# cocowy1/PPMStereo

Hardware: AMD Instinct MI355X
Metric: disparity-px/s (higher is better)
Workload: dtype bf16; 1 GPU; BASELINE config 2: T=5 clip at 320x512, iters=10, hot path only (3-scale cascade from encoder outputs: corr pyramid build + lookup, QAM pick, pick-and-play memory attention, ConvGRU3D update, heads, convex upsample, test_mode=True as PPMStereo.forward_batch_test calls it: predictions[-1] is the output, so the mask head, the convex upsampling and the full-resolution resize run only where their resu; T=5, H=320, W=512, iters=10, parallelism=replicas x1

## Files before the change

### include/ppms.h

```cpp
#ifndef PPMS_H
#define PPMS_H
#include <stdint.h>

#ifdef __cplusplus
extern "C" {
#endif

#define PPMS_OK 0
#define PPMS_EINVAL (-1)
#define PPMS_ELAUNCH (-2)
#define PPMS_ENODEV (-3)

#define PPMS_ABI_VERSION 4

int ppms_version(void);
const char* ppms_last_error(void);
int ppms_device_info(char* name, int name_cap, int* cu_count, int* clock_mhz);

int ppms_corr_build(const float* fmap1, const float* fmap2, float* const pyr[5], int B, int C, int H, int W, void* stream);

int ppms_corr_lookup(const float* const pyr[4], const float* flow, int flow_nhwc, float* out_nchw, void* out_hi, void* out_lo,
                     int out_ld, void* flow_sp_hi, void* flow_sp_lo, int flow_sp_ld, int B, int H, int W, void* stream);

typedef struct ppms_sp {
// ... 42 lines not shown
    int32_t lo_zero_from;
    ppms_epilogue epi[2];
} ppms_conv;

int ppms_conv_gemm2(const ppms_conv* desc, const ppms_conv* dev_desc, int wm_hint, void* stream);
int ppms_conv_gemm2_slices(const ppms_conv* desc);
int64_t ppms_conv_gemm2_slice_workspace_bytes(const ppms_conv* desc, int nslice);
int ppms_conv_gemm2_sliced(const ppms_conv* desc, const ppms_conv* dev_desc, int nslice, void* workspace, void* stream);
int ppms_conv_gemm2_ysweep_slices(const ppms_conv* desc);
int ppms_conv_gemm2_ysweep(const ppms_conv* desc, const ppms_conv* dev_desc, int nslice, void* workspace, void* stream);
int ppms_conv_gemm5_applicable(const ppms_conv* desc);
int ppms_conv_gemm5(const ppms_conv* desc, const ppms_conv* dev_desc, int nbt, void* stream);
int ppms_conv_gemm5_slices(const ppms_conv* desc);
int ppms_conv_gemm5_sliced(const ppms_conv* desc, const ppms_conv* dev_desc, int nbt, int nslice, void* workspace, void* stream);
int ppms_conv_gemm6_applicable(const ppms_conv* desc);
int ppms_conv_gemm6(const ppms_conv* desc, const ppms_conv* dev_desc, void* stream);
int ppms_gemm1_applicable(const ppms_conv* desc);
int ppms_gemm1(const ppms_conv* desc, const ppms_conv* dev_desc, int cb_hint, void* stream);
int ppms_conv_stream_applicable(const ppms_conv* desc);
int ppms_conv_stream(const ppms_conv* desc, const ppms_conv* dev_desc, int hint, void* stream);
int ppms_struct_sizes(int* sp, int* epilogue, int* conv);

int ppms_dwconv_gelu(ppms_sp x, ppms_sp y, const float* w, const float* b, int k, int BT, int H, int W, void* stream);
int ppms_flow_patch7(const float* flow_nhwc, ppms_sp patch, int BT, int H, int W, void* stream);
int ppms_unc_tail(ppms_sp x, const float* w, float bias, float* unc, float* partial, int BT, int HW, void* stream);

int ppms_nchw_to_sp(const float* src, ppms_sp dst, int BT, int C, int HW, void* stream);
int ppms_sp_to_nchw(ppms_sp src, float* dst, int BT, int C, int HW, void* stream);
int ppms_nchw_to_nhwc(const float* src, float* dst, int dst_ld, int BT, int C, int HW, void* stream);
int ppms_nhwc_to_nchw(const float* src, int src_ld, float* dst, int BT, int C, int HW, void* stream);
int ppms_f32_to_sp(const float* src, int src_ld, ppms_sp dst, int64_t pixels, void* stream);
int ppms_sp_to_f32(ppms_sp src, float* dst, int dst_ld, int64_t pixels, void* stream);

int ppms_tap_gather_sum(const float* y, int y_ld, const float* bias, float* out, int out_ld, float* accum, int accum_ld, int cout, int kt, int kh,
                        int kw, int T, int H, int W, int t_halo, void* stream);
int ppms_flow_add(float* flow_nhwc, const float* dflow, int dflow_ld, int64_t pixels, void* stream);
int ppms_convex_upsample(const float* flow_nhwc, const float* mask, int mask_ld, float* out, int BT, int H, int W, void* stream);
int ppms_convex_upsample_3d(const float* flow_nhwc, const float* mask, int mask_ld, float* out, int T, int H, int W, int t_halo, void* stream);
int ppms_bilinear(const float* src, float* dst, int N, int C, int H, int W, int OH, int OW, int align_corners, float mul, void* stream);

int ppms_sp_resize_blend(ppms_sp src, ppms_sp dst, int N, int H, int W, int OH, int OW, float a, float b, void* stream);

int ppms_avgpool(const float* src, float* dst, int planes, int H, int W, int k, void* stream);
int ppms_axpby(const float* x, const float* y, float* out, float a, float b, int64_t period, int64_t n, void* stream);
int ppms_ctx_mix(const float* fmap, const float* ctx, float* net, float* inp, int N, int HW, void* stream);

int ppms_img_s2d(const float* img_nchw, ppms_sp dst, int N, int C, int H, int W, int k, void* stream);
int ppms_sp_s2d(ppms_sp src, ppms_sp dst, int N, int H, int W, void* stream);
int ppms_video_ingest_u8(const uint8_t* left, const uint8_t* right, int64_t frame_stride, int N, int H0, int W0, int pad_left, int pad_top, int H, int W,
                         const float* lut, ppms_sp dst_fnet, ppms_sp dst_cnet, void* stream);
int64_t ppms_instnorm_workspace_bytes(int N, int HW, int C);
int ppms_instnorm_stats(const float* x, int ld, int N, int HW, int C, float eps, float* stats, void* workspace, void* stream);
int ppms_instnorm_apply(const float* x, int ld, const float* stats, ppms_sp res, int relu, ppms_sp out, int N, int HW, int C, void* stream);

int ppms_dwconv(ppms_sp x, float* y, int ldy, const float* w, const float* b, int k, int N, int H, int W, void* stream);
int ppms_layernorm_any(const float* x, int ld, const float* w, const float* b, float eps, ppms_sp out, int64_t pixels, int C, void* stream);
int64_t ppms_grn_workspace_bytes(int N, int HW, int C);
int ppms_grn(const float* x, int ld, const float* gamma, const float* beta, ppms_sp out, int N, int HW, int C, void* workspace, void* stream);
int ppms_sp_upsample2(ppms_sp src, ppms_sp dst, int N, int H, int W, void* stream);

int ppms_qk_similarity(const float* q, const float* k, int ld, float* pooled, float* sim, int T, int H, int W, void* stream);
int ppms_qk_pool(const float* q, const float* k, int ld, float* pooled, int T, int H, int W, void* stream);
int ppms_qk_cos(const float* pooled, float* sim, int T, int cells, void* stream);
int ppms_qam_select(const float* sim, float* strive, const float* conf_partial, int nblk, int HW, int32_t* sel, float* shat,
                    float* score, int T, void* stream);
int ppms_attn_prep_q(const float* q, int ld, const float* pe, void* qb, int T, int n, void* stream);
int ppms_attn_prep_k(const float* key, int ld, const float* pe, const int32_t* sel, const float* shat, void* kb, int T, int ksel,
                     int n, void* stream);
enum { PPMS_ATTN_P_BF16 = 0, PPMS_ATTN_P_FP16 = 1 };
int ppms_mem_attn(const void* qb, const void* kb, const void* vt, const int32_t* sel, int ksel, float scale, const float* beta,
                  ppms_sp mf, ppms_sp mfg, void* out_bf16, int T, int n, void* split_ws, int frames_per_workgroup, int p_format, void* stream);
int64_t ppms_mem_attn_workspace_bytes(int T, int ksel, int n);
int ppms_mem_attn_splits(int T, int ksel, int n, int frames_per_workgroup);
int ppms_attn_redo_accumulate(const void* split_ws, int T, int ksel, int n, int frames_per_workgroup, int64_t* counters, void* stream);

int ppms_pwchain(const void* dev_params, int64_t pixels, void* stream);
int ppms_pwchain_param_bytes(void);

int ppms_time_attn(ppms_sp x, const float* ln_w, const float* ln_b, ppms_sp out, int T, int n, int heads, void* stream);
int ppms_layernorm(const float* x, int ld, const float* w, const float* b, ppms_sp resid, ppms_sp out, int64_t pixels, int C, void* stream);
int64_t ppms_linear_attention_workspace_floats(int T, int n, int heads, int dh);
int ppms_linear_attention(const float* Q, int ldq, const float* K, int ldk, const float* V, int ldv, float* kv_ws, ppms_sp out, int T, int n,
                          int heads, int dh, void* stream);

#ifdef __cplusplus
}
#endif
#endif
```

### ppmstereo_amd/_lib.py

```python
from __future__ import annotations

import ctypes as C
import os
from typing import Optional

import torch

from . import build as _build

c_void_p, c_int, c_float, c_int64 = C.c_void_p, C.c_int, C.c_float, C.c_int64

EPI_STORE, EPI_RESID, EPI_RH, EPI_GRU, EPI_ADDF32 = range(5)
ATTN_P_BF16, ATTN_P_FP16 = 0, 1
ACT_NONE, ACT_RELU, ACT_GELU, ACT_SIGMOID, ACT_TANH, ACT_ELU1 = range(6)


def vt_image(v: torch.Tensor, p_format: int) -> torch.Tensor:
    b = v.to(torch.bfloat16)
    if p_format == ATTN_P_BF16:
        return b.contiguous()
    return b.float().clamp(-65504.0, 65504.0).to(torch.float16).contiguous().view(torch.bfloat16)


def vt_values(vt: torch.Tensor, p_format: int) -> torch.Tensor:
# ... 32 lines not shown
    "ppms_last_error": (C.c_char_p, []),
    "ppms_device_info": (c_int, [C.c_char_p, c_int, C.POINTER(c_int), C.POINTER(c_int)]),
    "ppms_corr_build": (c_int, [c_void_p, c_void_p, C.POINTER(c_void_p), c_int, c_int, c_int, c_int, c_void_p]),
    "ppms_corr_lookup": (c_int, [C.POINTER(c_void_p), c_void_p, c_int, c_void_p, c_void_p, c_void_p, c_int, c_void_p, c_void_p,
                                 c_int, c_int, c_int, c_int, c_void_p]),
    "ppms_conv_gemm2": (c_int, [C.POINTER(Conv), c_void_p, c_int, c_void_p]),
    "ppms_conv_gemm2_slices": (c_int, [C.POINTER(Conv)]),
    "ppms_conv_gemm2_slice_workspace_bytes": (C.c_int64, [C.POINTER(Conv), c_int]),
    "ppms_conv_gemm2_sliced": (c_int, [C.POINTER(Conv), c_void_p, c_int, c_void_p, c_void_p]),
    "ppms_conv_gemm2_ysweep_slices": (c_int, [C.POINTER(Conv)]),
    "ppms_conv_gemm2_ysweep": (c_int, [C.POINTER(Conv), c_void_p, c_int, c_void_p, c_void_p]),
    "ppms_gemm1_applicable": (c_int, [C.POINTER(Conv)]),
    "ppms_gemm1": (c_int, [C.POINTER(Conv), c_void_p, c_int, c_void_p]),
    "ppms_conv_stream_applicable": (c_int, [C.POINTER(Conv)]),
    "ppms_conv_stream": (c_int, [C.POINTER(Conv), c_void_p, c_int, c_void_p]),
    "ppms_conv_gemm5_applicable": (c_int, [C.POINTER(Conv)]),
    "ppms_conv_gemm5": (c_int, [C.POINTER(Conv), c_void_p, c_int, c_void_p]),
    "ppms_conv_gemm6_applicable": (c_int, [C.POINTER(Conv)]),
    "ppms_conv_gemm6": (c_int, [C.POINTER(Conv), c_void_p, c_void_p]),
    "ppms_conv_gemm5_slices": (c_int, [C.POINTER(Conv)]),
    "ppms_conv_gemm5_sliced": (c_int, [C.POINTER(Conv), c_void_p, c_int, c_int, c_void_p, c_void_p]),
    "ppms_struct_sizes": (c_int, [C.POINTER(c_int), C.POINTER(c_int), C.POINTER(c_int)]),
    "ppms_dwconv_gelu": (c_int, [SP, SP, c_void_p, c_void_p, c_int, c_int, c_int, c_int, c_void_p]),
    "ppms_flow_patch7": (c_int, [c_void_p, SP, c_int, c_int, c_int, c_void_p]),
    "ppms_unc_tail": (c_int, [SP, c_void_p, c_float, c_void_p, c_void_p, c_int, c_int, c_void_p]),
    "ppms_nchw_to_sp": (c_int, [c_void_p, SP, c_int, c_int, c_int, c_void_p]),
    "ppms_sp_to_nchw": (c_int, [SP, c_void_p, c_int, c_int, c_int, c_void_p]),
    "ppms_nchw_to_nhwc": (c_int, [c_void_p, c_void_p, c_int, c_int, c_int, c_int, c_void_p]),
    "ppms_nhwc_to_nchw": (c_int, [c_void_p, c_int, c_void_p, c_int, c_int, c_int, c_void_p]),
    "ppms_f32_to_sp": (c_int, [c_void_p, c_int, SP, c_int64, c_void_p]),
    "ppms_sp_to_f32": (c_int, [SP, c_void_p, c_int, c_int64, c_void_p]),
    "ppms_tap_gather_sum": (c_int, [c_void_p, c_int, c_void_p, c_void_p, c_int, c_void_p, c_int, c_int, c_int, c_int, c_int, c_int, c_int, c_int, c_int, c_void_p]),
    "ppms_flow_add": (c_int, [c_void_p, c_void_p, c_int, c_int64, c_void_p]),
    "ppms_convex_upsample": (c_int, [c_void_p, c_void_p, c_int, c_void_p, c_int, c_int, c_int, c_void_p]),
    "ppms_convex_upsample_3d": (c_int, [c_void_p, c_void_p, c_int, c_void_p, c_int, c_int, c_int, c_int, c_void_p]),
    "ppms_bilinear": (c_int, [c_void_p, c_void_p, c_int, c_int, c_int, c_int, c_int, c_int, c_int, c_float, c_void_p]),
    "ppms_sp_resize_blend": (c_int, [SP, SP, c_int, c_int, c_int, c_int, c_int, c_float, c_float, c_void_p]),
    "ppms_avgpool": (c_int, [c_void_p, c_void_p, c_int, c_int, c_int, c_int, c_void_p]),
    "ppms_axpby": (c_int, [c_void_p, c_void_p, c_void_p, c_float, c_float, c_int64, c_int64, c_void_p]),
    "ppms_ctx_mix": (c_int, [c_void_p, c_void_p, c_void_p, c_void_p, c_int, c_int, c_void_p]),
    "ppms_img_s2d": (c_int, [c_void_p, SP, c_int, c_int, c_int, c_int, c_int, c_void_p]),
    "ppms_video_ingest_u8": (c_int, [c_void_p, c_void_p, c_int64, c_int, c_int, c_int, c_int, c_int, c_int, c_int, c_void_p, SP, SP, c_void_p]),
    "ppms_dwconv": (c_int, [SP, c_void_p, c_int, c_void_p, c_void_p, c_int, c_int, c_int, c_int, c_void_p]),
    "ppms_layernorm_any": (c_int, [c_void_p, c_int, c_void_p, c_void_p, c_float, SP, c_int64, c_int, c_void_p]),
    "ppms_grn_workspace_bytes": (c_int64, [c_int, c_int, c_int]),
    "ppms_grn": (c_int, [c_void_p, c_int, c_void_p, c_void_p, SP, c_int, c_int, c_int, c_void_p, c_void_p]),
    "ppms_sp_upsample2": (c_int, [SP, SP, c_int, c_int, c_int, c_void_p]),
    "ppms_sp_s2d": (c_int, [SP, SP, c_int, c_int, c_int, c_void_p]),
    "ppms_instnorm_workspace_bytes": (c_int64, [c_int, c_int, c_int]),
    "ppms_instnorm_stats": (c_int, [c_void_p, c_int, c_int, c_int, c_int, C.c_float, c_void_p, c_void_p, c_void_p]),
    "ppms_instnorm_apply": (c_int, [c_void_p, c_int, c_void_p, SP, c_int, SP, c_int, c_int, c_int, c_void_p]),
    "ppms_qk_similarity": (c_int, [c_void_p, c_void_p, c_int, c_void_p, c_void_p, c_int, c_int, c_int, c_void_p]),
    "ppms_qk_pool": (c_int, [c_void_p, c_void_p, c_int, c_void_p, c_int, c_int, c_int, c_void_p]),
    "ppms_qk_cos": (c_int, [c_void_p, c_void_p, c_int, c_int, c_void_p]),
    "ppms_qam_select": (c_int, [c_void_p, c_void_p, c_void_p, c_int, c_int, c_void_p, c_void_p, c_void_p, c_int, c_void_p]),
    "ppms_attn_prep_q": (c_int, [c_void_p, c_int, c_void_p, c_void_p, c_int, c_int, c_void_p]),
    "ppms_attn_prep_k": (c_int, [c_void_p, c_int, c_void_p, c_void_p, c_void_p, c_void_p, c_int, c_int, c_int, c_void_p]),
    "ppms_pwchain": (c_int, [c_void_p, c_int64, c_void_p]),
    "ppms_pwchain_param_bytes": (c_int, []),
    "ppms_time_attn": (c_int, [SP, c_void_p, c_void_p, SP, c_int, c_int, c_int, c_void_p]),
    "ppms_layernorm": (c_int, [c_void_p, c_int, c_void_p, c_void_p, SP, SP, c_int64, c_int, c_void_p]),
    "ppms_linear_attention_workspace_floats": (c_int64, [c_int, c_int, c_int, c_int]),
    "ppms_linear_attention": (c_int, [c_void_p, c_int, c_void_p, c_int, c_void_p, c_int, c_void_p, SP, c_int, c_int, c_int, c_int, c_void_p]),
    "ppms_mem_attn": (c_int, [c_void_p, c_void_p, c_void_p, c_void_p, c_int, c_float, c_void_p, SP, SP, c_void_p, c_int, c_int, c_void_p, c_int, c_int, c_void_p]),
    "ppms_mem_attn_workspace_bytes": (c_int64, [c_int, c_int, c_int]),
    "ppms_mem_attn_splits": (c_int, [c_int, c_int, c_int, c_int]),
    "ppms_attn_redo_accumulate": (c_int, [c_void_p, c_int, c_int, c_int, c_int, c_void_p, c_void_p]),
}
EXPORTS = tuple(_SIGS)

_lib: Optional[C.CDLL] = None


def lib_path() -> str:
    return _build.LIB


def load() -> C.CDLL:
    global _lib
    if _lib is not None:
# ... 71 lines not shown
```

### ppmstereo_amd/csrc/small_ops.hip

```cpp
#include "common.h"

static thread_local char g_err[512] = "";
void ppms_set_error(const char* fmt, ...) {
    va_list ap;
    va_start(ap, fmt);
    vsnprintf(g_err, sizeof(g_err), fmt, ap);
    va_end(ap);
}
int ppms_check_launch(const char* what) {
    hipError_t e = hipGetLastError();
    if (e != hipSuccess) {
        ppms_set_error("%s: HIP launch failed: %s", what, hipGetErrorString(e));
        return PPMS_ELAUNCH;
    }
    return PPMS_OK;
}
extern "C" const char* ppms_last_error(void) { return g_err; }
extern "C" int ppms_version(void) { return PPMS_ABI_VERSION; }
extern "C" int ppms_struct_sizes(int* sp, int* epilogue, int* conv) {
    if (sp) *sp = (int)sizeof(ppms_sp);
    if (epilogue) *epilogue = (int)sizeof(ppms_epilogue);
    if (conv) *conv = (int)sizeof(ppms_conv);
    return PPMS_OK;
}
// ... 76 lines not shown
            const f32x4 w0 = *(const f32x4*)(wl + (ky * K + kx) * C + c0), w1 = *(const f32x4*)(wl + (ky * K + kx) * C + c0 + 4);
#pragma unroll
            for (int p = 0; p < DW_PX; ++p)
#pragma unroll
                for (int j = 0; j < 8; ++j) acc[p][j] += (j < 4 ? w0[j & 3] : w1[j & 3]) * win[p + kx][j];
        }
    }
#pragma unroll
    for (int p = 0; p < DW_PX; ++p) {
        if (px0 + p >= W) break;
        bf16x8 oh, ol;
#pragma unroll
        for (int j = 0; j < 8; ++j) {
            bf16_t hi, lo;
            split_bf16(gelu_erf(x0[p][j] + acc[p][j]), hi, lo);
            oh[j] = hi;
            ol[j] = lo;
        }
        *(bf16x8*)((bf16_t*)y.hi + (pix0 + p) * y.ld + c0) = oh;
        *(bf16x8*)((bf16_t*)y.lo + (pix0 + p) * y.ld + c0) = ol;
    }
}

extern "C" int ppms_dwconv_gelu(ppms_sp x, ppms_sp y, const float* w, const float* b, int k, int BT, int H, int W, void* stream) {
    PPMS_REQUIRE(k == 1 || k == 7, "dwconv_gelu: k=%d (only 1 and 7)", k);
    PPMS_REQUIRE(x.hi && x.lo && y.hi && y.lo && x.c == y.c && x.c > 0 && x.c <= 64 && x.c % 8 == 0 && x.ld % 8 == 0 && y.ld % 8 == 0,
                 "dwconv_gelu: views must have c <= 64 and c, ld multiples of 8");
    const int64_t rows = (int64_t)BT * H;
    const int groups = x.c / 8;
    const dim3 grid(ceil_div(rows * ((W + DW_PX - 1) / DW_PX) * groups, 256));
    if (k == 1)
        hipLaunchKernelGGL(dwconv_gelu_kernel<1>, grid, dim3(256), 0, (hipStream_t)stream, x, y, w, b, H, W, rows, groups);
    else
        hipLaunchKernelGGL(dwconv_gelu_kernel<7>, grid, dim3(256), 0, (hipStream_t)stream, x, y, w, b, H, W, rows, groups);
    return ppms_check_launch("dwconv_gelu");
}

__global__ __launch_bounds__(256) void flow_patch7_kernel(const float* __restrict__ flow, ppms_sp patch, int H, int W, int64_t P) {
    const int64_t idx = (int64_t)blockIdx.x * 256 + threadIdx.x;
    if (idx >= P * 128) return;
    const int k = (int)(idx & 127);
    const int64_t pix = idx >> 7;
    float v = 0.0f;
    if (k < 98) {
        const int tap = k >> 1, c = k & 1;
        const int ky = tap / 7, kx = tap - ky * 7;
        const int px = (int)(pix % W), py = (int)((pix / W) % H);
        const int xx = px + kx - 3, yy = py + ky - 3;
        if ((unsigned)xx < (unsigned)W && (unsigned)yy < (unsigned)H) v = flow[(pix + (int64_t)(ky - 3) * W + (kx - 3)) * 2 + c];
    }
    bf16_t hi, lo;
    split_bf16(v, hi, lo);
    ((bf16_t*)patch.hi)[pix * patch.ld + k] = hi;
    ((bf16_t*)patch.lo)[pix * patch.ld + k] = lo;
}

extern "C" int ppms_flow_patch7(const float* flow_nhwc, ppms_sp patch, int BT, int H, int W, void* stream) {
    PPMS_REQUIRE(flow_nhwc && patch.hi && patch.lo && patch.ld >= 128, "flow_patch7: bad arguments");
// ... 616 lines not shown
    const int cs = (int)(r / n);
    const int clip = cs / ksel, slot = cs - clip * ksel;
    const int frame = sel[clip * 5 + slot];
    const float s = shat[clip * 5 + slot];
    const float* kp = key + ((int64_t)frame * n + pin) * ld + g * 8;
    const f32x4 a = *(const f32x4*)kp, b = *(const f32x4*)(kp + 4);
    const f32x4 pa = *(const f32x4*)(pe + frame * 128 + g * 8), pb = *(const f32x4*)(pe + frame * 128 + g * 8 + 4);
    bf16x8 o;
#pragma unroll
    for (int j = 0; j < 4; ++j) {
        o[j] = (bf16_t)(a[j] * s + pa[j]);
        o[4 + j] = (bf16_t)(b[j] * s + pb[j]);
    }
    *(bf16x8*)(kb + r * 128 + g * 8) = o;
}
extern "C" int ppms_attn_prep_k(const float* key, int ld, const float* pe, const int32_t* sel, const float* shat, void* kb, int T, int ksel,
                                int n, void* stream) {
    PPMS_REQUIRE(key && pe && sel && shat && kb && ksel >= 1 && ksel <= 5 && ld % 4 == 0, "attn_prep_k: bad arguments");
    const int64_t total = (int64_t)T * ksel * n * 16;
    hipLaunchKernelGGL(attn_prep_k_kernel, dim3(ceil_div(total, 256)), dim3(256), 0, (hipStream_t)stream, key, ld, pe, sel, shat,
                       (bf16_t*)kb, ksel, n, total);
    return ppms_check_launch("attn_prep_k");
}
```

### ppmstereo_amd/engine.py

```python
from __future__ import annotations

import ctypes as C
import math
from typing import Dict, List, Optional

import torch

from . import _lib as L
from . import packing as _packing
from .convplan import (ALL_KERNELS, CONV2, CONV2_SWEPT, CONV6, KERNEL_TIMING, TUNING, ConvOp, PwChain, TimedCall,
                       attn_p_format, conv_desc, epilogue, pack_conv, plan_conv)

TOP_K = 5


def temporal_pe(T: int, channels: int) -> torch.Tensor:
    pos = torch.arange(T)
    pos = pos / pos[-1] * 1.0
    pos = pos.unsqueeze(1)
    div = 1.0 / (10000.0 ** (torch.arange(0, channels, 2).float() / channels))
    ang = pos * div
    pe = torch.zeros(T, channels)
    pe[:, 0::2] = torch.sin(ang)
    pe[:, 1::2] = torch.cos(ang)
# ... 9 lines not shown
    def __init__(self, sd: Dict[str, torch.Tensor], device):
        g = lambda k: sd[k].detach().to(device=device, dtype=torch.float32)
        self.w: Dict[str, dict] = {}

        def put(name, weight, bias, segs, seg_pad=None, cout_map=None, m_pad=None, kernels=ALL_KERNELS):
            self.w[name] = pack_conv(weight, bias, segs, seg_pad, cout_map, m_pad, kernels)

        e = "encoder."
        put("init0", g(e + "init_conv.0.weight"), g(e + "init_conv.0.bias"), [128])
        put("init2", g(e + "init_conv.2.weight"), g(e + "init_conv.2.bias"), [64])
        c1 = e + "convc1."
        put("ffn1_0", g(c1 + "ffn1.0.weight"), g(c1 + "ffn1.0.bias"), [36], [64], kernels=(CONV2,))
        put("ffn1_2", g(c1 + "ffn1.2.weight"), g(c1 + "ffn1.2.bias"), [54], [64], kernels=(CONV2,))
        put("pw", g(c1 + "pw.weight"), g(c1 + "pw.bias"), [36], [64], kernels=(CONV2,))
        put("ffn2_0", g(c1 + "ffn2.0.weight"), g(c1 + "ffn2.0.bias"), [36], [64], kernels=(CONV2,))
        put("ffn2_2", g(c1 + "ffn2.2.weight"), g(c1 + "ffn2.2.bias"), [54], [64], kernels=(CONV2,))
        self.dw = []
        for i, k in ((0, 1), (1, 7)):
            w = torch.zeros(64, k * k, device=device)
            b = torch.zeros(64, device=device)
            w[:36] = g(c1 + f"conv_list.{i}.weight").reshape(36, k * k)
            b[:36] = g(c1 + f"conv_list.{i}.bias")
            self.dw.append((w.contiguous(), b.contiguous(), k))
        put("convc2", g(e + "convc2.weight"), g(e + "convc2.bias"), [256])
        wf1 = g(e + "convf1.weight").permute(0, 2, 3, 1).reshape(128, 98, 1, 1)
        put("convf1", wf1, g(e + "convf1.bias"), [98], [128])
        put("convf2", g(e + "convf2.weight"), g(e + "convf2.bias"), [128])
        put("final", g(e + "final_conv.weight"), g(e + "final_conv.bias"), [320], None, list(range(126)) + list(range(128, 192)), 192)
        put("to_v", g("aggregator.to_v.weight"), None, [128])
        put("unc0", g("uncertainty.0.weight"), g("uncertainty.0.bias"), [128, 128])
        self.unc2_w = g("uncertainty.2.weight").reshape(128).contiguous()
        self.unc2_b = float(sd["uncertainty.2.bias"].detach().float().cpu().item())
        gr = "gru."
        cat = lambda a, b: torch.cat([g(a), g(b)], 0)
        put("zr1_0", cat(gr + "convz1.0.weight", gr + "convr1.0.weight"), cat(gr + "convz1.0.bias", gr + "convr1.0.bias"), [128, 384])
        put("z1_2", g(gr + "convz1.2.weight"), g(gr + "convz1.2.bias"), [128])
        put("r1_2", g(gr + "convr1.2.weight"), g(gr + "convr1.2.bias"), [128])
        self.w["zr1_2"] = {CONV6: _packing.pack_conv6_grouped([g(gr + "convz1.2.weight"), g(gr + "convr1.2.weight")], [g(gr + "convz1.2.bias"), g(gr + "convr1.2.bias")], 128)}
        put("q1", g(gr + "convq1.weight"), g(gr + "convq1.bias"), [128, 384])
        for n in ("2", "3"):
            put("zr" + n, cat(gr + f"convz{n}.weight", gr + f"convr{n}.weight"), cat(gr + f"convz{n}.bias", gr + f"convr{n}.bias"), [128, 384])
            put("q" + n, g(gr + f"convq{n}.weight"), g(gr + f"convq{n}.bias"), [128, 384])
        self.hoist = "time_attn.temporal_fc.weight" not in sd
        if self.hoist:
            for name in ("zr1_0", "q1", "zr2", "q2", "zr3", "q3"):
                if name.startswith("zr"):
# ... 66 lines not shown
            self.XG = self.X if shard is None else L.SPTensor(Tg * n, 384, device)
            self.QKF, self.VF, self.M2, self.M3 = f32(P, 768), f32(P, 384), f32(P, 384), f32(P, 384)
            self.KVWS = f32(int(L.load().ppms_linear_attention_workspace_floats(T, n, 8, 48)))
        self.Hb = [sp(128), sp(128), sp(128)]
        self.ZT, self.RT, self.RH, self.FH1, self.M1 = sp(128), sp(128), sp(128), sp(256), sp(256)
        self.Z, self.MASK, self.QK = f32(P, 128), f32(P, pk.mask_ch), f32(P, 256)
        self._FLOW_full, self._FH2Y_full = f32(P + 2 * hp, 2), f32(P + 2 * hp, 64)
        self.FLOW, self.FH2Y = self._FLOW_full[hp:hp + P], self._FH2Y_full[hp:hp + P]
        self.DFLOW = f32(P, 4)
        if pk.hoist:
            self.PRE = {k: torch.empty(P, m, dtype=torch.float32, device=device) for k, m in
                        (("zr1_0", 256), ("q1", 128), ("zr2", 256), ("q2", 128), ("zr3", 256), ("q3", 128))}
            self._pre_stream, self._ev_pre, self._pre_pending = torch.cuda.Stream(device=device), torch.cuda.Event(), False
        self.attn_p = attn_p_format()
        self.VT = torch.zeros(T, 128, n, dtype=torch.bfloat16, device=device)
        self.VTG = self.VT if shard is None else torch.zeros(Tg, 128, n, dtype=torch.bfloat16, device=device)
        self.KG = None if shard is None else f32(Tg * n, 128)
        self.QB = torch.zeros(T, n, 128, dtype=torch.bfloat16, device=device)
        self.KB = torch.zeros(T, self.ksel, n, 128, dtype=torch.bfloat16, device=device)
        self.ATT_WS = torch.empty(int(L.load().ppms_mem_attn_workspace_bytes(T, self.ksel, n)), dtype=torch.uint8, device=device)
        self.nblk = (n + 255) // 256
        self.UNC, self.PART = f32(P), f32(T, self.nblk)
        self.PARTG = self.PART if shard is None else f32(Tg, self.nblk)
        self.SIM, self.STRIVE, self.SCORE = f32(Tg, Tg), f32(Tg, Tg), f32(Tg, Tg)
        self.SEL = torch.zeros(Tg, 5, dtype=torch.int32, device=device)
        self.SHAT = f32(Tg, 5)
        self.cells = max(1, (h // 4) * (w // 4))
        self.POOL = f32(2, T, self.cells)
        self.POOLG = self.POOL if shard is None else f32(2, Tg, self.cells)
        self.PE = temporal_pe(Tg, 128).to(device)
        self.FLOW_OUT = f32(T, 2, 4 * h, 4 * w)
        self.scale = softmax_scale(128)
        self.parity = 0
        self.have_mhs = False
        self.lib = L.load()
        self._ev, self._ev_i = None, 0
        self._health, self._health_on = None, False
        self._xa_halo = None
        self._x_hid = False
        self.hbm = {"corr_lookup": TimedCall(self._lookup), "attn_prep_k": TimedCall(self._prep_k), "convex_upsample": TimedCall(self._upsample)}
        self._side = torch.cuda.Stream(device=device)
        self._ev_fork, self._ev_join = torch.cuda.Event(), torch.cuda.Event()
        self._build_descriptors()

    def _halo_sp(self, tensors, k: int, async_op: bool = False):
        if self.shard is None:
            return None
        if isinstance(tensors, L.SPTensor):
            tensors = [tensors]
        fr = self.T + 2 * self.halo
        return self.shard.halo_many([(t.data[p].view(fr, self.n, t.channels), k) for t in tensors for p in (0, 1)], async_op)

    def _halo_f32(self, full: torch.Tensor, k: int):
        if self.shard is not None:
            self.shard.halo(full.view(self.T + 2 * self.halo, self.n, full.shape[1]), k)

    def _conv(self, packs, segs: List[L.SP], k3, epi0: L.Epilogue, epi1: Optional[L.Epilogue] = None, m_split: int = 0, keep=(),
              lo_zero_from: int = 0) -> ConvOp:
        d = conv_desc(segs, (self.T, self.h, self.w), k3, epi0, epi1, m_split, self.halo if k3[0] > 1 else 0, lo_zero_from)
        return plan_conv(d, self.pk.w[packs] if isinstance(packs, str) else packs, keep, device=self.dev)

    def _build_descriptors(self):
        E, X, H = epilogue, self.X, self.Hb
        k1, k3 = (1, 1, 1), (1, 3, 3)
        inp, mf, mfg = X.view(0, 128), X.view(128, 128), X.view(256, 128)
        self.op: Dict[str, object] = {}
        o = self.op
        self._qk_ops: Dict[int, ConvOp] = {}
        o["init0"] = self._conv("init0", [inp], k3, E(act=L.ACT_RELU, n_valid=64, out_sp=self.ZT.view(0, 64)))
        w = {k: self.pk.w[k][CONV2] for k in ("ffn1_0", "ffn1_2", "pw", "ffn2_0", "ffn2_2")}
        (w1, b1, _), (w7, b7, _) = self.pk.dw
        dw1 = (w1.reshape(64).contiguous(), b1)
        o["chainA"] = PwChain(self.CORR.view(), self.C2.view(), [(w["ffn1_0"], 54, False, None), (w["ffn1_2"], 36, True, dw1)], self.P, [dw1[0]],
                             device=self.dev)
        o["chainB"] = PwChain(self.C1.view(), self.COR256.view(), [(w["pw"], 36, True, None), (w["ffn2_0"], 54, False, None),
                                                                   (w["ffn2_2"], 256, False, None)], self.P, [], device=self.dev)
        o["dw7"] = TimedCall(lambda: L.check(self.lib.ppms_dwconv_gelu(self.C2.view(0, 40), self.C1.view(0, 40), w7.data_ptr(), b7.data_ptr(), 7,
                                                                        self.T, self.h, self.w, L.stream_ptr())))
        o["convf1"] = self._conv("convf1", [self.PATCH.view()], k1, E(act=L.ACT_RELU, n_valid=128, out_sp=self.FLO1.view()))
        for par in (0, 1):
            cf, cf_next = self.CF[par], self.CF[1 - par]
            o[f"init2_{par}"] = self._conv("init2", [self.ZT.view(0, 64)], k3, E(n_valid=64, out_sp=cf.view(256, 64)))
            o[f"convc2_{par}"] = self._conv("convc2", [self.COR256.view()], k3, E(act=L.ACT_RELU, n_valid=192, out_sp=cf.view(0, 192)))
            o[f"convf2_{par}"] = self._conv("convf2", [self.FLO1.view()], k3, E(act=L.ACT_RELU, n_valid=64, out_sp=cf.view(192, 64)))
            o[f"final_{par}"] = self._conv("final", [cf.view()], k3, E(act=L.ACT_RELU, n_valid=126, out_sp=mf),
                                           E(act=L.ACT_RELU, n_valid=64, out_sp=cf_next.view(256, 64)), m_split=128)
        o["to_v"] = self._conv("to_v", [mf], k1, E(n_valid=128, out_sp=self.VAL.view(), out_vt=self.VT, vt_f16=self.attn_p))
        o["unc0"] = self._conv("unc0", [H[0].view(), self.VAL.view()], k3, E(act=L.ACT_RELU, n_valid=128, out_sp=self.U1.view()))
        if self.pk.attn is not None:
            o["ta_fc"] = self._conv("ta_fc", [self.O1.view()], k1, E(L.EPI_RESID, n_valid=384, out_sp=self.XT.view(), aux_sp=X.view()))
            o["sa_qkv"] = self._conv("sa_qkv", [self.XT.view()], k1, E(act=L.ACT_ELU1, n_valid=768, out_f32=self.QKF, out_f32_ld=768),
                                     E(scale=1.0 / self.n, n_valid=384, out_f32=self.VF, out_f32_ld=384), m_split=768)
            o["sa_merge"] = self._conv("sa_merge", [self.MSG.view()], k1, E(n_valid=384, out_f32=self.M2, out_f32_ld=384))
            o["sa_mlp0"] = self._conv("sa_mlp0", [self.XT.view(), self.MSGN.view()], k1, E(act=L.ACT_RELU, n_valid=768, out_sp=self.H1.view()))
            o["sa_mlp2"] = self._conv("sa_mlp2", [self.H1.view()], k1, E(n_valid=384, out_f32=self.M3, out_f32_ld=384))
        x_all = self.XA.view()
        hoist = self.pk.hoist
        if hoist:
            x_all = X.view(128, 256)
            for k, kk in (("zr1_0", (1, 1, 15)), ("q1", (1, 1, 5)), ("zr2", (1, 5, 1)), ("q2", (1, 5, 1)), ("zr3", (5, 1, 1)), ("q3", (5, 1, 1))):
                m = self.PRE[k].shape[1]
# ... 101 lines not shown
            mfg = self.X.to_f32(128, 128) + self.pk.beta * self.X.to_f32(256, 128)
            return mfg.reshape(self.T, self.h, self.w, 128).permute(0, 3, 1, 2).contiguous()
        return self.store_nchw(self.X.view(256, 128), 128)

    def get_value(self):
        return self.store_nchw(self.VAL.view(), 128)

    def get_flow(self):
        out = torch.empty(self.T, 2, self.h, self.w, dtype=torch.float32, device=self.dev)
        L.check(self.lib.ppms_nhwc_to_nchw(self.FLOW.data_ptr(), 2, out.data_ptr(), self.T, 2, self.n, self._s()))
        return out

    def get_dflow(self):
        out = torch.empty(self.T, 2, self.h, self.w, dtype=torch.float32, device=self.dev)
        L.check(self.lib.ppms_nhwc_to_nchw(self.DFLOW.data_ptr(), 4, out.data_ptr(), self.T, 2, self.n, self._s()))
        return out

    def get_mask(self):
        mc = self.pk.mask_ch
        out = torch.empty(self.T, mc, self.h, self.w, dtype=torch.float32, device=self.dev)
        L.check(self.lib.ppms_nhwc_to_nchw(self.MASK.data_ptr(), mc, out.data_ptr(), self.T, mc, self.n, self._s()))
        return out

    def get_unc(self):
        return self.UNC.view(self.T, 1, self.h, self.w).clone()

    def begin(self, pyramid: List[torch.Tensor], qk_pack):
        self._drain_xa_halo()
        self.pyr = pyramid
        self.pyr_ptrs = (C.c_void_p * 4)(*[p.data_ptr() for p in pyramid[:4]])
        self.qk_op(qk_pack)()
        s = self._s()
        pe_local = self.PE.data_ptr() + self.f0 * 128 * 4
        L.check(self.lib.ppms_attn_prep_q(self.QK.data_ptr(), 256, pe_local, self.QB.data_ptr(), self.T, self.n, s))
        L.check(self.lib.ppms_qk_pool(self.QK.data_ptr(), self.QK.data_ptr() + 128 * 4, 256, self.POOL.data_ptr(), self.T, self.h, self.w, s))
        if self.shard is not None:
            g, _ = self.shard.all_gather(self.POOL.permute(1, 0, 2).contiguous())
            self.POOLG.copy_(g.permute(1, 0, 2))
            self.shard.all_gather(self.QK[:, 128:].contiguous(), out=self.KG)
        L.check(self.lib.ppms_qk_cos(self.POOLG.data_ptr(), self.SIM.data_ptr(), self.Tg, self.cells, s))
        self.STRIVE.fill_(1.0)

    def qk_op(self, qk_pack) -> ConvOp:
        key = qk_pack[CONV2][0].data_ptr()
        if key not in self._qk_ops:
            self._qk_ops[key] = self._conv(qk_pack, [self.X.view(0, 128)], (1, 1, 1), epilogue(n_valid=256, out_f32=self.QK, out_f32_ld=256))
# ... 33 lines not shown
            o["init0"]()
            o[f"init2_{par}"]()
            self.have_mhs = True
        o["chainA"]()
        o["dw7"]()
        o["chainB"]()
        o[f"convc2_{par}"]()
        self._join()
        o[f"final_{par}"]()
        self.parity = 1 - par
        o["to_v"]()

    def uncertainty(self):
        self.op["unc0"]()
        L.check(self.lib.ppms_unc_tail(self.U1.view(), self.pk.unc2_w.data_ptr(), self.pk.unc2_b, self.UNC.data_ptr(), self.PART.data_ptr(),
                                       self.T, self.n, self._s()))

    def pick(self):
        if self.shard is not None:
            self.shard.gather_many([(self.VT, self.VTG), (self.PART, self.PARTG)])
        L.check(self.lib.ppms_qam_select(self.SIM.data_ptr(), self.STRIVE.data_ptr(), self.PARTG.data_ptr(), self.nblk, self.n, self.SEL.data_ptr(),
                                         self.SHAT.data_ptr(), self.SCORE.data_ptr(), self.Tg, self._s()))

    def attend(self, out_bf16: Optional[torch.Tensor] = None):
        s = self._s()
        sel = self.SEL.data_ptr() + self.f0 * 5 * 4
        shat = self.SHAT.data_ptr() + self.f0 * 5 * 4
        if self.shard is None:
            key, key_ld = self.QK.data_ptr() + 128 * 4, 256
        else:
            key, key_ld = self.KG.data_ptr(), 128
        self._prep_k_args = (key, key_ld, sel, shat)
        self.hbm["attn_prep_k"]()
        ev = None
        if KERNEL_TIMING["on"] and self._ev is not None and self._ev_i < len(self._ev):
            ev = self._ev[self._ev_i]
            self._ev_i += 1
            ev[0].record()
        mf_in = L.SP(None, None, 0, 0) if self.hid_mode else self.X.view(128, 128)
        L.check(self.lib.ppms_mem_attn(self.QB.data_ptr(), self.KB.data_ptr(), self.VTG.data_ptr(), sel, self.ksel, self.scale,
                                       self.pk.beta.data_ptr(), mf_in, self.X.view(256, 128), L.ptr(out_bf16), self.T, self.n,
                                       self.ATT_WS.data_ptr(), 0, self.attn_p, s))
        if self._health_on:
            L.check(self.lib.ppms_attn_redo_accumulate(self.ATT_WS.data_ptr(), self.T, self.ksel, self.n, 0, self._health.data_ptr(), s))
        self._x_hid = self.hid_mode
        if ev is not None:
            ev[1].record()
        if self.shard is not None and self.pk.attn is None:
# ... 91 lines not shown
                self._halo_sp(self.XA, 2)
        o["zr3" + tag]()
        self._halo_sp(self.RH, 2)
        o["q3" + tag]()
        self._halo_sp(self.Hb[0], 1)
        if need_mask:
            with self._fork():
                o["m1"]()
                o["m2"]()
        o["fh1"]()
        o["fh2"]()
        self._halo_f32(self._FH2Y_full, 1)
        L.check(self.lib.ppms_tap_gather_sum(self.FH2Y.data_ptr(), 64, self.pk.fh2_bias.data_ptr(), self.DFLOW.data_ptr(), 4, self.FLOW.data_ptr(), 2,
                                             2, 3, 3, 3, self.T, self.h, self.w, self.halo, self._s()))
        if need_mask:
            self._join()

    def upsample(self) -> torch.Tensor:
        self.hbm["convex_upsample"]()
        return self.FLOW_OUT

    def _prep_k(self):
        key, key_ld, sel, shat = self._prep_k_args
        L.check(self.lib.ppms_attn_prep_k(key, key_ld, self.PE.data_ptr(), sel, shat, self.KB.data_ptr(), self.T, self.ksel, self.n, self._s()))

    def _upsample(self):
        if self.pk.convex_3d:
            self._halo_f32(self._FLOW_full, 1)
            L.check(self.lib.ppms_convex_upsample_3d(self.FLOW.data_ptr(), self.MASK.data_ptr(), self.pk.mask_ch, self.FLOW_OUT.data_ptr(), self.T,
                                                     self.h, self.w, self.halo, self._s()))
        else:
            L.check(self.lib.ppms_convex_upsample(self.FLOW.data_ptr(), self.MASK.data_ptr(), self.pk.mask_ch, self.FLOW_OUT.data_ptr(), self.T,
                                                  self.h, self.w, self._s()))

    def iterate(self, need_up: bool = True):
        self.lookup()
        self.motion_and_value()
        self.uncertainty()
        self.pick()
        self.attend()
        self.update(need_mask=need_up)
        return self.upsample() if need_up else None


def bilinear(x: torch.Tensor, size, align_corners: bool, mul: float = 1.0) -> torch.Tensor:
    x = x.contiguous().float()
    L.require_gpu(x)
    N, Cc, H, W = x.shape
    out = torch.empty(N, Cc, size[0], size[1], dtype=torch.float32, device=x.device)
    L.check(L.load().ppms_bilinear(x.data_ptr(), out.data_ptr(), N, Cc, H, W, size[0], size[1], int(align_corners), mul, L.stream_ptr()))
    return out
```

Measured before the change: 23.54 million disparity-px/s.

## Tile 7x7 depthwise conv through LDS and fuse QAM pick into key prep

Replaces the direct 7x7 depthwise conv+GELU kernel with an LDS-tiled kernel that stages an input patch and tap-major weights in shared memory and computes several pixels per thread. Separately, the QAM frame selection is fused into the attention key-prep kernel, with a double-buffered strive state, so one launch and a global round trip of sel/shat are removed. The fused kernel recomputes the selection in every block, and the tiled conv uses more LDS and registers per thread.

```diff
diff --git a/include/ppms.h b/include/ppms.h
--- a/include/ppms.h
+++ b/include/ppms.h
@@ -88,6 +88,7 @@
 int ppms_struct_sizes(int* sp, int* epilogue, int* conv);
 
 int ppms_dwconv_gelu(ppms_sp x, ppms_sp y, const float* w, const float* b, int k, int BT, int H, int W, void* stream);
+int ppms_dwconv_gelu_tm(ppms_sp x, ppms_sp y, const float* w_tapmajor, const float* b, int BT, int H, int W, void* stream);
 int ppms_flow_patch7(const float* flow_nhwc, ppms_sp patch, int BT, int H, int W, void* stream);
 int ppms_unc_tail(ppms_sp x, const float* w, float bias, float* unc, float* partial, int BT, int HW, void* stream);
 
@@ -133,6 +134,9 @@
 int ppms_attn_prep_q(const float* q, int ld, const float* pe, void* qb, int T, int n, void* stream);
 int ppms_attn_prep_k(const float* key, int ld, const float* pe, const int32_t* sel, const float* shat, void* kb, int T, int ksel,
                      int n, void* stream);
+int ppms_attn_pick_prep_k(const float* key, int ld, const float* pe, const float* sim, const float* strive_in, float* strive_out,
+                          const float* conf_partial, int nblk, int HW, int32_t* sel, float* shat, float* score, void* kb, int T, int ksel,
+                          int n, void* stream);
 enum { PPMS_ATTN_P_BF16 = 0, PPMS_ATTN_P_FP16 = 1 };
 int ppms_mem_attn(const void* qb, const void* kb, const void* vt, const int32_t* sel, int ksel, float scale, const float* beta,
                   ppms_sp mf, ppms_sp mfg, void* out_bf16, int T, int n, void* split_ws, int frames_per_workgroup, int p_format, void* stream);
diff --git a/ppmstereo_amd/_lib.py b/ppmstereo_amd/_lib.py
--- a/ppmstereo_amd/_lib.py
+++ b/ppmstereo_amd/_lib.py
@@ -78,6 +78,7 @@
     "ppms_conv_gemm5_sliced": (c_int, [C.POINTER(Conv), c_void_p, c_int, c_int, c_void_p, c_void_p]),
     "ppms_struct_sizes": (c_int, [C.POINTER(c_int), C.POINTER(c_int), C.POINTER(c_int)]),
     "ppms_dwconv_gelu": (c_int, [SP, SP, c_void_p, c_void_p, c_int, c_int, c_int, c_int, c_void_p]),
+    "ppms_dwconv_gelu_tm": (c_int, [SP, SP, c_void_p, c_void_p, c_int, c_int, c_int, c_void_p]),
     "ppms_flow_patch7": (c_int, [c_void_p, SP, c_int, c_int, c_int, c_void_p]),
     "ppms_unc_tail": (c_int, [SP, c_void_p, c_float, c_void_p, c_void_p, c_int, c_int, c_void_p]),
     "ppms_nchw_to_sp": (c_int, [c_void_p, SP, c_int, c_int, c_int, c_void_p]),
@@ -112,6 +113,8 @@
     "ppms_qam_select": (c_int, [c_void_p, c_void_p, c_void_p, c_int, c_int, c_void_p, c_void_p, c_void_p, c_int, c_void_p]),
     "ppms_attn_prep_q": (c_int, [c_void_p, c_int, c_void_p, c_void_p, c_int, c_int, c_void_p]),
     "ppms_attn_prep_k": (c_int, [c_void_p, c_int, c_void_p, c_void_p, c_void_p, c_void_p, c_int, c_int, c_int, c_void_p]),
+    "ppms_attn_pick_prep_k": (c_int, [c_void_p, c_int, c_void_p, c_void_p, c_void_p, c_void_p, c_void_p, c_int, c_int, c_void_p, c_void_p, c_void_p,
+                                      c_void_p, c_int, c_int, c_int, c_void_p]),
     "ppms_pwchain": (c_int, [c_void_p, c_int64, c_void_p]),
     "ppms_pwchain_param_bytes": (c_int, []),
     "ppms_time_attn": (c_int, [SP, c_void_p, c_void_p, SP, c_int, c_int, c_int, c_void_p]),
diff --git a/ppmstereo_amd/csrc/small_ops.hip b/ppmstereo_amd/csrc/small_ops.hip
--- a/ppmstereo_amd/csrc/small_ops.hip
+++ b/ppmstereo_amd/csrc/small_ops.hip
@@ -122,18 +122,155 @@
     }
 }
 
+struct dw_tile {
+    int th, tw, gpb, ngb, tiles_x, tiles_y, rs;
+};
+template <int PX, bool TAPMAJOR>
+__global__ __launch_bounds__(512) void dwconv7_tiled_kernel(ppms_sp x, ppms_sp y, const float* __restrict__ w, const float* __restrict__ b,
+                                                            int H, int W, int groups, dw_tile t) {
+    extern __shared__ __attribute__((aligned(16))) f32x4 dw_lds[];
+    constexpr int K = 7, R = 3, NW = PX + K - 1;
+    const int gpb = t.gpb, PH = t.th + 2 * R, PW = t.tw + 2 * R, rpr = t.tw / PX;
+    const int gb = blockIdx.x % t.ngb, tile = blockIdx.x / t.ngb;
+    const int tx = tile % t.tiles_x, ty = (tile / t.tiles_x) % t.tiles_y, frame = tile / (t.tiles_x * t.tiles_y);
+    const int g0 = gb * gpb, ng = min(gpb, groups - g0);
+    f32x4* wl = dw_lds;
+    f32x4* patch = dw_lds + K * K * 2 * gpb;
+    {
+        float* wf = (float*)wl;
+        const int nc = ng * 8, C = groups * 8;
+        for (int i = threadIdx.x; i < K * K * nc; i += blockDim.x) {
+            const int cc = i % nc, tap = i / nc, c = g0 * 8 + cc;
+            wf[((tap * 2 + ((cc >> 2) & 1)) * gpb + (cc >> 3)) * 4 + (cc & 3)] = TAPMAJOR ? w[tap * C + c] : w[c * K * K + tap];
+        }
+    }
+    const int y0 = ty * t.th - R, x0g = tx * t.tw - R;
+    for (int i = threadIdx.x; i < PH * PW * ng; i += blockDim.x) {
+        const int g = i % ng, pp = i / ng, pxp = pp % PW, prow = pp / PW;
+        const int gy = y0 + prow, gx = x0g + pxp;
+        f32x4 v0 = {0.0f, 0.0f, 0.0f, 0.0f}, v1 = v0;
+        if ((unsigned)gy < (unsigned)H && (unsigned)gx < (unsigned)W) {
+            const int64_t q = ((int64_t)frame * H + gy) * W + gx;
+            const bf16x8 h8 = *(const bf16x8*)((const bf16_t*)x.hi + q * x.ld + (g0 + g) * 8);
+            const bf16x8 l8 = *(const bf16x8*)((const bf16_t*)x.lo + q * x.ld + (g0 + g) * 8);
+#pragma unroll
+            for (int j = 0; j < 4; ++j) {
+                v0[j] = join_bf16(h8[j], l8[j]);
+                v1[j] = join_bf16(h8[4 + j], l8[4 + j]);
+            }
+        }
+        const int s = ((pxp % PX) * PH + prow) * t.rs + (pxp / PX) * gpb + g;
+        patch[s] = v0;
+        patch[PX * PH * t.rs + s] = v1;
+    }
+    __syncthreads();
+    const int g = threadIdx.x % gpb, run = (threadIdx.x / gpb) % rpr, row = threadIdx.x / (gpb * rpr);
+    const int py = ty * t.th + row, px0 = tx * t.tw + run * PX;
+    if (g >= ng || row >= t.th || py >= H || px0 >= W) return;
+    const int c0 = (g0 + g) * 8;
+    float acc[PX][8], xc[PX][8];
+    {
+        const f32x4 b0 = *(const f32x4*)(b + c0), b1 = *(const f32x4*)(b + c0 + 4);
+#pragma unroll
+        for (int p = 0; p < PX; ++p)
+#pragma unroll
+            for (int j = 0; j < 8; ++j) acc[p][j] = j < 4 ? b0[j & 3] : b1[j & 3];
+    }
+    const f32x4* pl = patch + run * gpb + g;
+#pragma unroll 1
+    for (int ky = 0; ky < K; ++ky) {
+        float win[NW][8];
+#pragma unroll
+        for (int i = 0; i < NW; ++i) {
+            const int s = ((i % PX) * PH + row + ky) * t.rs + (i / PX) * gpb;
+            const f32x4 v0 = pl[s], v1 = pl[PX * PH * t.rs + s];
+#pragma unroll
+            for (int j = 0; j < 4; ++j) {
+                win[i][j] = v0[j];
+                win[i][4 + j] = v1[j];
+            }
+        }
+        if (ky == R) {
+#pragma unroll
+            for (int p = 0; p < PX; ++p)
+#pragma unroll
+                for (int j = 0; j < 8; ++j) xc[p][j] = win[p + R][j];
+        }
+#pragma unroll
+        for (int kx = 0; kx < K; ++kx) {
+            const f32x4 w0 = wl[((ky * K + kx) * 2 + 0) * gpb + g], w1 = wl[((ky * K + kx) * 2 + 1) * gpb + g];
+#pragma unroll
+            for (int p = 0; p < PX; ++p)
+#pragma unroll
+                for (int j = 0; j < 8; ++j) acc[p][j] += (j < 4 ? w0[j & 3] : w1[j & 3]) * win[p + kx][j];
+        }
+    }
+    const int64_t pix0 = ((int64_t)frame * H + py) * W + px0;
+#pragma unroll
+    for (int p = 0; p < PX; ++p) {
+        if (px0 + p >= W) break;
+        bf16x8 oh, ol;
+#pragma unroll
+        for (int j = 0; j < 8; ++j) {
+            bf16_t hi, lo;
+            split_bf16(gelu_erf(xc[p][j] + acc[p][j]), hi, lo);
+            oh[j] = hi;
+            ol[j] = lo;
+        }
+        *(bf16x8*)((bf16_t*)y.hi + (pix0 + p) * y.ld + c0) = oh;
+        *(bf16x8*)((bf16_t*)y.lo + (pix0 + p) * y.ld + c0) = ol;
+    }
+}
+
+static int dwconv7_launch(ppms_sp x, ppms_sp y, const float* w, const float* b, bool tapmajor, int BT, int H, int W, hipStream_t stream) {
+    const int groups = x.c / 8;
+    const bool large = (int64_t)BT * H * W >= 4096;
+    dw_tile t;
+    t.th = 8;
+    t.tw = large ? 16 : 8;
+    const int px = large ? 2 : 1;
+    t.tiles_x = ceil_div(W, t.tw);
+    t.tiles_y = ceil_div(H, t.th);
+    const int64_t tiles = (int64_t)BT * t.tiles_x * t.tiles_y;
+    if (large) {
+        const int want = (int)std::min<int64_t>(groups, std::max<int64_t>(ceil_div(groups, 5), ceil_div(256, tiles)));
+        t.gpb = ceil_div(groups, want);
+    } else {
+        t.gpb = 1;
+    }
+    t.ngb = ceil_div(groups, t.gpb);
+    const int lanes_per_row = (t.tw / px) * t.gpb;
+    const int rs0 = ceil_div(t.tw + 6, px) * t.gpb;
+    t.rs = rs0 + (((lanes_per_row - rs0) % 16) + 16) % 16;
+    const int threads = ceil_div(t.th * lanes_per_row, 64) * 64;
+    const size_t lds = (size_t)(49 * 2 * t.gpb + 2 * px * (t.th + 6) * t.rs) * 16;
+    PPMS_REQUIRE(tiles * t.ngb < (1ll << 31) && threads <= 512 && lds <= 64 * 1024, "dwconv_gelu: %d x %d x %d does not fit the tiled kernel", BT, H, W);
+    const dim3 grid((unsigned)(tiles * t.ngb));
+    if (large && tapmajor)
+        hipLaunchKernelGGL((dwconv7_tiled_kernel<2, true>), grid, dim3(threads), lds, stream, x, y, w, b, H, W, groups, t);
+    else if (large)
+        hipLaunchKernelGGL((dwconv7_tiled_kernel<2, false>), grid, dim3(threads), lds, stream, x, y, w, b, H, W, groups, t);
+    else if (tapmajor)
+        hipLaunchKernelGGL((dwconv7_tiled_kernel<1, true>), grid, dim3(threads), lds, stream, x, y, w, b, H, W, groups, t);
+    else
+        hipLaunchKernelGGL((dwconv7_tiled_kernel<1, false>), grid, dim3(threads), lds, stream, x, y, w, b, H, W, groups, t);
+    return ppms_check_launch("dwconv_gelu");
+}
+
+#define PPMS_DWCONV_VIEWS_OK (x.hi && x.lo && y.hi && y.lo && x.c == y.c && x.c > 0 && x.c <= 64 && x.c % 8 == 0 && x.ld % 8 == 0 && y.ld % 8 == 0)
 extern "C" int ppms_dwconv_gelu(ppms_sp x, ppms_sp y, const float* w, const float* b, int k, int BT, int H, int W, void* stream) {
     PPMS_REQUIRE(k == 1 || k == 7, "dwconv_gelu: k=%d (only 1 and 7)", k);
-    PPMS_REQUIRE(x.hi && x.lo && y.hi && y.lo && x.c == y.c && x.c > 0 && x.c <= 64 && x.c % 8 == 0 && x.ld % 8 == 0 && y.ld % 8 == 0,
-                 "dwconv_gelu: views must have c <= 64 and c, ld multiples of 8");
+    PPMS_REQUIRE(PPMS_DWCONV_VIEWS_OK, "dwconv_gelu: views must have c <= 64 and c, ld multiples of 8");
+    if (k == 7) return dwconv7_launch(x, y, w, b, false, BT, H, W, (hipStream_t)stream);
     const int64_t rows = (int64_t)BT * H;
     const int groups = x.c / 8;
     const dim3 grid(ceil_div(rows * ((W + DW_PX - 1) / DW_PX) * groups, 256));
-    if (k == 1)
-        hipLaunchKernelGGL(dwconv_gelu_kernel<1>, grid, dim3(256), 0, (hipStream_t)stream, x, y, w, b, H, W, rows, groups);
-    else
-        hipLaunchKernelGGL(dwconv_gelu_kernel<7>, grid, dim3(256), 0, (hipStream_t)stream, x, y, w, b, H, W, rows, groups);
+    hipLaunchKernelGGL(dwconv_gelu_kernel<1>, grid, dim3(256), 0, (hipStream_t)stream, x, y, w, b, H, W, rows, groups);
     return ppms_check_launch("dwconv_gelu");
+}
+extern "C" int ppms_dwconv_gelu_tm(ppms_sp x, ppms_sp y, const float* w_tapmajor, const float* b, int BT, int H, int W, void* stream) {
+    PPMS_REQUIRE(PPMS_DWCONV_VIEWS_OK && w_tapmajor && b, "dwconv_gelu_tm: views must have c <= 64 and c, ld multiples of 8");
+    return dwconv7_launch(x, y, w_tapmajor, b, true, BT, H, W, (hipStream_t)stream);
 }
 
 __global__ __launch_bounds__(256) void flow_patch7_kernel(const float* __restrict__ flow, ppms_sp patch, int H, int W, int64_t P) {
@@ -796,3 +933,107 @@
                        (bf16_t*)kb, ksel, n, total);
     return ppms_check_launch("attn_prep_k");
 }
+
+struct pick_lds {
+    int32_t sel[5];
+    float shat[5];
+};
+__global__ __launch_bounds__(256) void attn_pick_prep_k_kernel(const float* __restrict__ key, int ld, const float* __restrict__ pe,
+                                                               const float* __restrict__ sim, const float* __restrict__ strive_in,
+                                                               float* __restrict__ strive_out, const float* __restrict__ partial, int nblk, int HW,
+                                                               int32_t* __restrict__ sel_out, float* __restrict__ shat_out,
+                                                               float* __restrict__ score_out, bf16_t* __restrict__ kb, int T, int ksel, int n) {
+    __shared__ pick_lds pk;
+    const int i = blockIdx.y;
+    if (threadIdx.x < 64) {
+        const int lane = threadIdx.x;
+        float conf = 0.0f;
+        for (int f = 0; f < T; ++f) {
+            float s = 0.0f;
+            for (int bl = lane; bl < nblk; bl += 64) s += partial[f * nblk + bl];
+#pragma unroll
+            for (int m = 32; m >= 1; m >>= 1) s += __shfl_xor(s, m);
+            if (lane == f) conf = s / (float)HW;
+        }
+        float ssum = 0.0f;
+        for (int j = 0; j < T; ++j) ssum += strive_in[i * T + j];
+        float sc = 0.0f, used = 0.0f;
+        if (lane < T) {
+            used = strive_in[i * T + lane];
+            const float pen = expf(-used / (ssum + (float)T));
+            sc = pen * sim[i * T + lane] + conf;
+        }
+        unsigned long long picked = 0ull;
+        for (int r = 0; r < ksel; ++r) {
+            int best = -1;
+            float bv = -INFINITY;
+            for (int j = 0; j < T; ++j) {
+                if ((picked >> j) & 1ull) continue;
+                const float v = __shfl(sc, j);
+                if (best < 0 || v > bv || (v != v && bv == bv)) {
+                    best = j;
+                    bv = v;
+                }
+            }
+            picked |= 1ull << best;
+        }
+        float mean = 0.0f;
+        for (int j = 0; j < T; ++j)
+            if ((picked >> j) & 1ull) mean += __shfl(sc, j);
+        mean /= (float)ksel;
+        const bool owner = blockIdx.x == 0;
+        int r = 0;
+        for (int j = 0; j < T; ++j)
+            if ((picked >> j) & 1ull) {
+                const float sh = __shfl(sc, j) / mean;
+                if (lane == 0) {
+                    pk.sel[r] = j;
+                    pk.shat[r] = sh;
+                    if (owner) {
+                        sel_out[i * 5 + r] = j;
+                        shat_out[i * 5 + r] = sh;
+                    }
+                }
+                ++r;
+            }
+        if (owner && lane == 0)
+            for (; r < 5; ++r) {
+                sel_out[i * 5 + r] = 0;
+                shat_out[i * 5 + r] = 0.0f;
+            }
+        if (owner && lane < T) {
+            strive_out[i * T + lane] = ((picked >> lane) & 1ull) ? used + 1.0f : used;
+            if (score_out) score_out[i * T + lane] = sc;
+        }
+    }
+    __syncthreads();
+    const int64_t per_clip = (int64_t)ksel * n * 16;
+    for (int64_t e = (int64_t)blockIdx.x * 256 + threadIdx.x; e < per_clip; e += (int64_t)gridDim.x * 256) {
+        const int g = (int)(e & 15);
+        const int64_t rl = e >> 4;
+        const int slot = (int)(rl / n), pin = (int)(rl - (int64_t)slot * n);
+        const int frame = pk.sel[slot];
+        const float s = pk.shat[slot];
+        const float* kp = key + ((int64_t)frame * n + pin) * ld + g * 8;
+        const f32x4 a = *(const f32x4*)kp, b = *(const f32x4*)(kp + 4);
+        const f32x4 pa = *(const f32x4*)(pe + frame * 128 + g * 8), pb = *(const f32x4*)(pe + frame * 128 + g * 8 + 4);
+        bf16x8 o;
+#pragma unroll
+        for (int j = 0; j < 4; ++j) {
+            o[j] = (bf16_t)(a[j] * s + pa[j]);
+            o[4 + j] = (bf16_t)(b[j] * s + pb[j]);
+        }
+        *(bf16x8*)(kb + ((int64_t)i * ksel * n + rl) * 128 + g * 8) = o;
+    }
+}
+extern "C" int ppms_attn_pick_prep_k(const float* key, int ld, const float* pe, const float* sim, const float* strive_in, float* strive_out,
+                                     const float* conf_partial, int nblk, int HW, int32_t* sel, float* shat, float* score, void* kb, int T, int ksel,
+                                     int n, void* stream) {
+    PPMS_REQUIRE(key && pe && sim && strive_in && strive_out && strive_in != strive_out && conf_partial && sel && shat && kb && ld % 4 == 0 && n > 0 &&
+                     nblk > 0 && T > 0 && T <= 64 && ksel == (T < 5 ? T : 5),
+                 "attn_pick_prep_k: bad arguments (1 <= T <= 64, ksel = min(T, 5), strive_in != strive_out)");
+    const int bpc = (int)std::min<int64_t>(ceil_div((int64_t)ksel * n * 16, 256), std::max(1, 2048 / T));
+    hipLaunchKernelGGL(attn_pick_prep_k_kernel, dim3(bpc, T), dim3(256), 0, (hipStream_t)stream, key, ld, pe, sim, strive_in, strive_out,
+                       conf_partial, nblk, HW, sel, shat, score, (bf16_t*)kb, T, ksel, n);
+    return ppms_check_launch("attn_pick_prep_k");
+}
diff --git a/ppmstereo_amd/engine.py b/ppmstereo_amd/engine.py
--- a/ppmstereo_amd/engine.py
+++ b/ppmstereo_amd/engine.py
@@ -55,6 +55,7 @@
             w[:36] = g(c1 + f"conv_list.{i}.weight").reshape(36, k * k)
             b[:36] = g(c1 + f"conv_list.{i}.bias")
             self.dw.append((w.contiguous(), b.contiguous(), k))
+        self.dw7_tm = self.dw[1][0][:40].t().contiguous()
         put("convc2", g(e + "convc2.weight"), g(e + "convc2.bias"), [256])
         wf1 = g(e + "convf1.weight").permute(0, 2, 3, 1).reshape(128, 98, 1, 1)
         put("convf1", wf1, g(e + "convf1.bias"), [98], [128])
@@ -167,7 +168,8 @@
         self.nblk = (n + 255) // 256
         self.UNC, self.PART = f32(P), f32(T, self.nblk)
         self.PARTG = self.PART if shard is None else f32(Tg, self.nblk)
-        self.SIM, self.STRIVE, self.SCORE = f32(Tg, Tg), f32(Tg, Tg), f32(Tg, Tg)
+        self.SIM, self.SCORE = f32(Tg, Tg), f32(Tg, Tg)
+        self._strive, self._strive_i = (f32(Tg, Tg), f32(Tg, Tg)), 0
         self.SEL = torch.zeros(Tg, 5, dtype=torch.int32, device=device)
         self.SHAT = f32(Tg, 5)
         self.cells = max(1, (h // 4) * (w // 4))
@@ -182,6 +184,7 @@
         self._ev, self._ev_i = None, 0
         self._health, self._health_on = None, False
         self._xa_halo = None
+        self._fused_pick = False
         self._x_hid = False
         self.hbm = {"corr_lookup": TimedCall(self._lookup), "attn_prep_k": TimedCall(self._prep_k), "convex_upsample": TimedCall(self._upsample)}
         self._side = torch.cuda.Stream(device=device)
@@ -220,8 +223,9 @@
                              device=self.dev)
         o["chainB"] = PwChain(self.C1.view(), self.COR256.view(), [(w["pw"], 36, True, None), (w["ffn2_0"], 54, False, None),
                                                                    (w["ffn2_2"], 256, False, None)], self.P, [], device=self.dev)
-        o["dw7"] = TimedCall(lambda: L.check(self.lib.ppms_dwconv_gelu(self.C2.view(0, 40), self.C1.view(0, 40), w7.data_ptr(), b7.data_ptr(), 7,
-                                                                        self.T, self.h, self.w, L.stream_ptr())))
+        w7t = self.pk.dw7_tm
+        o["dw7"] = TimedCall(lambda: L.check(self.lib.ppms_dwconv_gelu_tm(self.C2.view(0, 40), self.C1.view(0, 40), w7t.data_ptr(), b7.data_ptr(),
+                                                                           self.T, self.h, self.w, L.stream_ptr())))
         o["convf1"] = self._conv("convf1", [self.PATCH.view()], k1, E(act=L.ACT_RELU, n_valid=128, out_sp=self.FLO1.view()))
         for par in (0, 1):
             cf, cf_next = self.CF[par], self.CF[1 - par]
@@ -369,6 +373,10 @@
         L.check(self.lib.ppms_nhwc_to_nchw(self.MASK.data_ptr(), mc, out.data_ptr(), self.T, mc, self.n, self._s()))
         return out
 
+    @property
+    def STRIVE(self) -> torch.Tensor:
+        return self._strive[self._strive_i]
+
     def get_unc(self):
         return self.UNC.view(self.T, 1, self.h, self.w).clone()
 
@@ -448,8 +456,11 @@
         L.check(self.lib.ppms_qam_select(self.SIM.data_ptr(), self.STRIVE.data_ptr(), self.PARTG.data_ptr(), self.nblk, self.n, self.SEL.data_ptr(),
                                          self.SHAT.data_ptr(), self.SCORE.data_ptr(), self.Tg, self._s()))
 
-    def attend(self, out_bf16: Optional[torch.Tensor] = None):
+    def attend(self, out_bf16: Optional[torch.Tensor] = None, pick: bool = False):
         s = self._s()
+        self._fused_pick = pick and self.shard is None
+        if pick and not self._fused_pick:
+            self.pick()
         sel = self.SEL.data_ptr() + self.f0 * 5 * 4
         shat = self.SHAT.data_ptr() + self.f0 * 5 * 4
         if self.shard is None:
@@ -587,6 +598,13 @@
 
     def _prep_k(self):
         key, key_ld, sel, shat = self._prep_k_args
+        if self._fused_pick:
+            src, dst = self._strive[self._strive_i], self._strive[1 - self._strive_i]
+            L.check(self.lib.ppms_attn_pick_prep_k(key, key_ld, self.PE.data_ptr(), self.SIM.data_ptr(), src.data_ptr(), dst.data_ptr(),
+                                                   self.PARTG.data_ptr(), self.nblk, self.n, sel, shat, self.SCORE.data_ptr(), self.KB.data_ptr(),
+                                                   self.T, self.ksel, self.n, self._s()))
+            self._strive_i = 1 - self._strive_i
+            return
         L.check(self.lib.ppms_attn_prep_k(key, key_ld, self.PE.data_ptr(), sel, shat, self.KB.data_ptr(), self.T, self.ksel, self.n, self._s()))
 
     def _upsample(self):
@@ -602,8 +620,7 @@
         self.lookup()
         self.motion_and_value()
         self.uncertainty()
-        self.pick()
-        self.attend()
+        self.attend(pick=True)
         self.update(need_mask=need_up)
         return self.upsample() if need_up else None
 
```

Measured after the change: 23.62 million disparity-px/s (median of 6 runs). No clear change (+0.3%).
